# ucuapps/OpenGlue

Hardware: NVIDIA H100
Metric: image-pairs/sec at N=M=2048, d=256, 9 GNN layers, 100 Sinkhorn iters (higher is better)
Workload: dtype fp16x3 (fp16 hi/lo operands with power-of-two tensor scales, 3 products, fp32 accumulate)

## Files before the change

openglue_b200/csrc/attention_sm90.cuh:

```cuda
#pragma once
#include "tc_common.cuh"
#include <math_constants.h>

namespace og {

struct TcAttnArgs {
  const float* q; int64_t ldq, strideq;
  float* out; int64_t ldo, strideo;
  int batch, nq, nk, num_heads, d;
  float scale;
  const int* klen;
};

struct F16AttnScales {
  const float* q_amax;
  const float* k_scale;
  const float* v_scale;
  float* out_amax;
  int swap_halves;
};

namespace tca {
constexpr int BM = 128;
constexpr float LOG2E = 1.4426950408889634f;
constexpr float P_SHIFT = 14.f;
template <int DH, bool F16> struct Cfg {
  static constexpr int ESZ = F16 ? 2 : 4;
  static constexpr int BOX = 128 / ESZ;
  static constexpr int BNK = F16 ? 128 : 64;
  static constexpr int THREADS = F16 ? 384 : 256;
  static constexpr int K_TILE = BNK * DH * ESZ;
  static constexpr int V_TILE = DH * BNK * ESZ;
  static constexpr int STAGE = 2 * K_TILE + 2 * V_TILE;
  static constexpr int STAGES = 3;
  static constexpr int SMEM_BYTES = 1024 + STAGES * STAGE + 128;
  static_assert(SMEM_BYTES <= OG_SMEM_OPTIN_MAX, "dynamic shared memory of one block");
};
}

template <int ROWS, int STEP_BYTES>
__device__ __forceinline__ uint64_t tile_desc(uint32_t tile, int kk) {
  const int byte = kk * STEP_BYTES;
  return tc::make_wgdesc_sw128(tile + (byte >> 7) * ROWS * 128 + (byte & 127));
}

template <int DH, bool F16>
__device__ __forceinline__ void attention_issue(uint8_t* st, uint64_t* full, const CUtensorMap* mkh, const CUtensorMap* mkl,
                                                const CUtensorMap* mvh, const CUtensorMap* mvl, const TcAttnArgs& a, int h, int b,
                                                int i) {
  using C = tca::Cfg<DH, F16>;
  tc::mbar_arrive_expect_tx(full, C::STAGE);
#pragma unroll
  for (int j = 0; j < DH / C::BOX; ++j) {
    tc::tma_load_2d(st + j * C::BNK * 128, mkh, full, h * DH + j * C::BOX, b * a.nk + i * C::BNK);
    tc::tma_load_2d(st + C::K_TILE + j * C::BNK * 128, mkl, full, h * DH + j * C::BOX, b * a.nk + i * C::BNK);
  }
#pragma unroll
  for (int j = 0; j < C::BNK / C::BOX; ++j) {
    tc::tma_load_2d(st + 2 * C::K_TILE + j * DH * 128, mvh, full, i * C::BNK + j * C::BOX, b * a.d + h * DH);
    tc::tma_load_2d(st + 2 * C::K_TILE + C::V_TILE + j * DH * 128, mvl, full, i * C::BNK + j * C::BOX, b * a.d + h * DH);
  }
}

template <int NJ, bool F16>
__device__ __forceinline__ void attention_softmax(float (&p)[4 * NJ], int k0, int t, int nk, float c1, float (&m_run)[2],
                                                  float (&mc_run)[2], float (&l_run)[2], float (&corr)[2]) {
  using namespace tca;
  if (k0 + 8 * NJ > nk) {
    const int kbase = k0 + 2 * t;
#pragma unroll
    for (int j = 0; j < NJ; ++j)
#pragma unroll
      for (int e = 0; e < 4; ++e) if (kbase + 8 * j + (e & 1) >= nk) p[4 * j + e] = -CUDART_INF_F;
  }
#pragma unroll
  for (int hh = 0; hh < 2; ++hh) {
    float mx = -CUDART_INF_F;
#pragma unroll
    for (int j = 0; j < NJ; ++j) mx = fmaxf(mx, fmaxf(p[4 * j + 2 * hh], p[4 * j + 2 * hh + 1]));
    mx = fmaxf(mx, __shfl_xor_sync(0xffffffffu, mx, 1));
    mx = fmaxf(mx, __shfl_xor_sync(0xffffffffu, mx, 2));
    const float m_new = fmaxf(m_run[hh], mx);
    const float mc = F16 ? fmaf(m_new, c1, -P_SHIFT) : m_new * c1;
    corr[hh] = ex2_approx(mc_run[hh] - mc);
    float r = 0.f;
#pragma unroll
    for (int j = 0; j < NJ; ++j) {
#pragma unroll
      for (int e = 0; e < 2; ++e) {
        float& x = p[4 * j + 2 * hh + e];
        x = ex2_approx(fmaf(x, c1, -mc));
        r += x;
      }
    }
    l_run[hh] = fmaf(l_run[hh], corr[hh], r);
    m_run[hh] = m_new; mc_run[hh] = mc;
  }
}

template <int DH>
__device__ __forceinline__ float attention_store(const float (&acc)[DH / 2], const float (&l_run)[2], float inv_sv, int qr, int t,
                                                 const TcAttnArgs& a, int h, int b) {
  float omax = 0.f;
#pragma unroll
  for (int hh = 0; hh < 2; ++hh) {
    float l = l_run[hh];
    l += __shfl_xor_sync(0xffffffffu, l, 1);
    l += __shfl_xor_sync(0xffffffffu, l, 2);
    const float inv = inv_sv / l;
    const int row = qr + 8 * hh;
    if (row >= a.nq) continue;
    float* orow = a.out + (int64_t)b * a.strideo + (int64_t)row * a.ldo + h * DH;
#pragma unroll
    for (int j = 0; j < DH / 8; ++j) {
      const float2 v = make_float2(acc[4 * j + 2 * hh] * inv, acc[4 * j + 2 * hh + 1] * inv);
      *reinterpret_cast<float2*>(orow + 8 * j + 2 * t) = v;
      omax = fmaxf(omax, fmaxf(fabsf(v.x), fabsf(v.y)));
    }
  }
  return omax;
}

template <int DH>
__device__ __forceinline__ void attention_f16_ws(const CUtensorMap* mkh, const CUtensorMap* mkl, const CUtensorMap* mvh,
                                                 const CUtensorMap* mvl, const TcAttnArgs& a, const F16AttnScales& sc,
                                                 uint8_t* smem) {
  using namespace tca;
  using namespace tc;
  using C = Cfg<DH, true>;
  constexpr int S = C::STAGES, BNK = C::BNK;
  constexpr int QK = DH / 16, PK = BNK / 16, NJ = BNK / 8;
  constexpr int TURN = 1;
  static_assert(DH * 2 == 128, "one 128-byte row per K row");
  uint64_t* full = reinterpret_cast<uint64_t*>(smem + S * C::STAGE);
  uint64_t* empty = full + S;
  volatile uint32_t* timeout_flag = reinterpret_cast<uint32_t*>(empty + S);

  const int q0 = blockIdx.x * BM, h = blockIdx.y, b = blockIdx.z;
  const int nk = padded_length(a.klen, b, a.nk);
  const int nblk = cdiv(nk, BNK);
  const int wg = threadIdx.x >> 7;
  if (threadIdx.x == 0) {
    for (int i = 0; i < S; ++i) { mbar_init(&full[i], 1); mbar_init(&empty[i], 2); }
    *timeout_flag = 0;
    fence_barrier_init();
    prefetch_tensormap(mkh); prefetch_tensormap(mkl);
    prefetch_tensormap(mvh); prefetch_tensormap(mvl);
  }
  __syncthreads();
  grid_dependency_wait();

  if (wg == 0) {
    setmaxnreg_dec<24>();
    if (threadIdx.x == 0) {
      for (int i = 0; i < nblk; ++i) {
        const int s = i % S;
        if (i >= S) mbar_wait(&empty[s], (i / S - 1) & 1);
        attention_issue<DH, true>(smem + s * C::STAGE, &full[s], mkh, mkl, mvh, mvl, a, h, b, i);
      }
      mbar_wait(&empty[(nblk - 1) % S], ((nblk - 1) / S) & 1);
      if (*timeout_flag) asm volatile("trap;");
    }
    return;
  }
  setmaxnreg_inc<240>();
  const int c = wg - 1, tid = threadIdx.x & 127, warp = tid >> 5, lane = tid & 31, g = lane >> 2, t = lane & 3;
  const float s_q = f16_scale_for(__ldcg(sc.q_amax));
  const float c1 = a.scale * LOG2E / (s_q * __ldcg(sc.k_scale));
  const float inv_sv = 1.f / __ldcg(sc.v_scale);

  const float* qb = a.q + (int64_t)b * a.strideq + h * DH;
  uint32_t qh[QK][4], ql[QK][4];
#pragma unroll
  for (int kk = 0; kk < QK; ++kk)
#pragma unroll
    for (int e = 0; e < 4; ++e) {
      const int grow = q0 + c * 64 + warp * 16 + g + (e & 1) * 8, col = kk * 16 + 2 * t + (e >> 1) * 8;
      const float2 v = grow < a.nq ? *reinterpret_cast<const float2*>(qb + (int64_t)grow * a.ldq + col) : make_float2(0.f, 0.f);
      split_f16x2(v.x * s_q, v.y * s_q, qh[kk][e], ql[kk][e]);
    }

  float acc[DH / 2], o[DH / 2], p[4 * NJ];
#pragma unroll
  for (int k = 0; k < DH / 2; ++k) acc[k] = 0.f;
  float m_run[2] = {-CUDART_INF_F, -CUDART_INF_F}, mc_run[2] = {-CUDART_INF_F, -CUDART_INF_F}, l_run[2] = {0.f, 0.f};
  float corr[2];
  uint32_t phi[PK][4], plo[PK][4];
  uint32_t timed_out = 0;

  auto issue_qk = [&](int s) {
    const uint32_t khi = smem_u32(smem + s * C::STAGE), klo = khi + C::K_TILE;
#pragma unroll
    for (int kk = 0; kk < QK; ++kk) {
      const uint64_t bh = tile_desc<BNK, 32>(khi, kk), bl = tile_desc<BNK, 32>(klo, kk);
      wgmma_f16_m64n128(p, ql[kk], bh, kk ? 1 : 0);
      wgmma_f16_m64n128(p, qh[kk], bl, 1);
      wgmma_f16_m64n128(p, qh[kk], bh, 1);
    }
  };
  auto issue_pv = [&](int s) {
    const uint32_t vhi = smem_u32(smem + s * C::STAGE) + 2 * C::K_TILE, vlo = vhi + C::V_TILE;
#pragma unroll
    for (int kk = 0; kk < PK; ++kk) {
      const uint64_t dhi = tile_desc<DH, 32>(vhi, kk), dlo = tile_desc<DH, 32>(vlo, kk);
      wgmma_f16_m64n64(o, plo[kk], dhi, kk ? 1 : 0);
      wgmma_f16_m64n64(o, phi[kk], dlo, 1);
      wgmma_f16_m64n64(o, phi[kk], dhi, 1);
    }
  };
  auto split_p = [&]() {
#pragma unroll
    for (int kk = 0; kk < PK; ++kk)
#pragma unroll
      for (int e = 0; e < 4; ++e) {
        const int base = 4 * (2 * kk + (e >> 1)) + 2 * (e & 1);
        split_f16x2(p[base], p[base + 1], phi[kk][e], plo[kk][e]);
        if (sc.swap_halves) { phi[kk][e] = __byte_perm(phi[kk][e], 0, 0x1032); plo[kk][e] = __byte_perm(plo[kk][e], 0, 0x1032); }
      }
  };
  auto release_and_fold = [&](int s) {
    if (tid == 0) mbar_arrive(&empty[s]);
#pragma unroll
    for (int k = 0; k < DH / 2; ++k) acc[k] = fmaf(acc[k], corr[(k >> 1) & 1], o[k]);
  };

  if (c == 1) named_bar_arrive(TURN + 0, 256);
  mbar_wait_flag(&full[0], 0, timed_out);
  named_bar_sync(TURN + c, 256);
  fence_operands(p);
  wgmma_fence();
  issue_qk(0);
  wgmma_commit();
  named_bar_arrive(TURN + (c ^ 1), 256);
  wgmma_wait<0>();
  fence_operands(p);
  attention_softmax<NJ, true>(p, 0, t, nk, c1, m_run, mc_run, l_run, corr);
  split_p();

#pragma unroll 1
  for (int i = 1; i < nblk; ++i) {
    const int s = i % S, sp = (i - 1) % S;
    mbar_wait_flag(&full[s], (i / S) & 1, timed_out);
    named_bar_sync(TURN + c, 256);
    fence_operands(p);
    fence_operands(o);
    wgmma_fence();
    issue_qk(s);
    issue_pv(sp);
    wgmma_commit();
    named_bar_arrive(TURN + (c ^ 1), 256);
    wgmma_wait<0>();
    fence_operands(p);
    fence_operands(o);
    release_and_fold(sp);
    attention_softmax<NJ, true>(p, i * BNK, t, nk, c1, m_run, mc_run, l_run, corr);
    split_p();
  }

  if (timed_out) *timeout_flag = 1;
  named_bar_sync(TURN + c, 256);
  fence_operands(o);
  wgmma_fence();
  issue_pv((nblk - 1) % S);
  wgmma_commit();
  if (c == 0) named_bar_arrive(TURN + 1, 256);
  wgmma_wait<0>();
  fence_operands(o);
  release_and_fold((nblk - 1) % S);

  float omax = attention_store<DH>(acc, l_run, inv_sv, q0 + c * 64 + warp * 16 + g, t, a, h, b);
  if (sc.out_amax) {
    omax = warp_max(omax);
    if (lane == 0 && omax > 0.f) atomic_amax(sc.out_amax, omax);
  }
}

template <int DH>
__device__ __forceinline__ void attention_tf32(const CUtensorMap* mkh, const CUtensorMap* mkl, const CUtensorMap* mvh,
                                               const CUtensorMap* mvl, const TcAttnArgs& a, uint8_t* smem) {
  using namespace tca;
  using namespace tc;
  using C = Cfg<DH, false>;
  constexpr int S = C::STAGES, BNK = C::BNK;
  constexpr int QK = DH / 8;
  uint64_t* full = reinterpret_cast<uint64_t*>(smem + S * C::STAGE);
  uint64_t* empty = full + S;

  const int q0 = blockIdx.x * BM, h = blockIdx.y, b = blockIdx.z;
  const int nk = padded_length(a.klen, b, a.nk);
  const int nblk = cdiv(nk, BNK);
  const int wg = threadIdx.x >> 7, warp = (threadIdx.x >> 5) & 3, lane = threadIdx.x & 31, g = lane >> 2, t = lane & 3;
  if (threadIdx.x == 0) {
    for (int i = 0; i < S; ++i) { mbar_init(&full[i], 1); mbar_init(&empty[i], 8); }
    fence_barrier_init();
    prefetch_tensormap(mkh); prefetch_tensormap(mkl);
    prefetch_tensormap(mvh); prefetch_tensormap(mvl);
  }
  __syncthreads();
  grid_dependency_wait();

  if (threadIdx.x == 0)
    for (int i = 0; i < S && i < nblk; ++i) attention_issue<DH, false>(smem + i * C::STAGE, &full[i], mkh, mkl, mvh, mvl, a, h, b, i);

  const int qr = q0 + wg * 64 + warp * 16 + g;
  const float c1 = a.scale * LOG2E;
  const float* qb = a.q + (int64_t)b * a.strideq + h * DH;
  uint32_t qhi[QK][4], qlo[QK][4];
#pragma unroll
  for (int kk = 0; kk < QK; ++kk) {
#pragma unroll
    for (int e = 0; e < 4; ++e) {
      const int row = qr + (e & 1) * 8;
      const int col = kk * 8 + t + (e >> 1) * 4;
      split_tf32(row < a.nq ? qb[(int64_t)row * a.ldq + col] : 0.f, qhi[kk][e], qlo[kk][e]);
    }
  }

  float acc[DH / 2];
#pragma unroll
  for (int k = 0; k < DH / 2; ++k) acc[k] = 0.f;
  float m_run[2] = {-CUDART_INF_F, -CUDART_INF_F}, mc_run[2] = {-CUDART_INF_F, -CUDART_INF_F}, l_run[2] = {0.f, 0.f};

#pragma unroll 1
  for (int i = 0; i < nblk; ++i) {
    if (threadIdx.x == 0 && i >= 1 && i - 1 + S < nblk) {
      const int sr = (i - 1) % S;
      mbar_wait(&empty[sr], ((i - 1) / S) & 1);
      attention_issue<DH, false>(smem + sr * C::STAGE, &full[sr], mkh, mkl, mvh, mvl, a, h, b, i - 1 + S);
    }
    const int s = i % S;
    mbar_wait(&full[s], (i / S) & 1);
    const uint32_t st = smem_u32(smem + s * C::STAGE);
    const uint32_t khi = st, klo = st + C::K_TILE, vhi = st + 2 * C::K_TILE, vlo = vhi + C::V_TILE;

    float p[32];
    fence_operands(p);
    wgmma_fence();
#pragma unroll
    for (int kk = 0; kk < QK; ++kk) {
      const uint64_t dhi = tile_desc<BNK, 32>(khi, kk), dlo = tile_desc<BNK, 32>(klo, kk);
      wgmma_tf32_m64n64(p, qlo[kk], dhi, kk ? 1 : 0);
      wgmma_tf32_m64n64(p, qhi[kk], dlo, 1);
      wgmma_tf32_m64n64(p, qhi[kk], dhi, 1);
    }
    wgmma_commit();
    wgmma_wait<0>();
    fence_operands(p);

    float corr[2];
    attention_softmax<8, false>(p, i * BNK, t, nk, c1, m_run, mc_run, l_run, corr);

    float o[DH / 2];
    const int src0 = (lane & ~3) | (t >> 1), src1 = src0 + 2;
    const bool odd = t & 1;
#pragma unroll
    for (int half = 0; half < 2; ++half) {
      uint32_t phi[4][4], plo[4][4];
#pragma unroll
      for (int jj = 0; jj < 4; ++jj) {
        const int j = half * 4 + jj;
#pragma unroll
        for (int e = 0; e < 4; ++e) {
          const int reg = 4 * j + 2 * (e & 1), src = (e >> 1) ? src1 : src0;
          const float x0 = __shfl_sync(0xffffffffu, p[reg], src), x1 = __shfl_sync(0xffffffffu, p[reg + 1], src);
          split_tf32(odd ? x1 : x0, phi[jj][e], plo[jj][e]);
        }
      }
      fence_operands(o);
      wgmma_fence();
#pragma unroll
      for (int jj = 0; jj < 4; ++jj) {
        const int kk = half * 4 + jj;
        const uint64_t dhi = tile_desc<DH, 32>(vhi, kk), dlo = tile_desc<DH, 32>(vlo, kk);
        if constexpr (DH == 64) {
          wgmma_tf32_m64n64(o, plo[jj], dhi, kk ? 1 : 0);
          wgmma_tf32_m64n64(o, phi[jj], dlo, 1);
          wgmma_tf32_m64n64(o, phi[jj], dhi, 1);
        } else {
          wgmma_tf32_m64n32(o, plo[jj], dhi, kk ? 1 : 0);
          wgmma_tf32_m64n32(o, phi[jj], dlo, 1);
          wgmma_tf32_m64n32(o, phi[jj], dhi, 1);
        }
      }
      wgmma_commit();
      wgmma_wait<0>();
      fence_operands(o);
    }
    __syncwarp();
    if (lane == 0) mbar_arrive(&empty[s]);
#pragma unroll
    for (int k = 0; k < DH / 2; ++k) acc[k] = fmaf(acc[k], corr[(k >> 1) & 1], o[k]);
  }
  attention_store<DH>(acc, l_run, 1.f, qr, t, a, h, b);
}

template <int DH, bool F16>
__global__ void __launch_bounds__(tca::Cfg<DH, F16>::THREADS, 1) attention_sm90_kernel(const __grid_constant__ CUtensorMap map_khi,
                                                                                       const __grid_constant__ CUtensorMap map_klo,
                                                                                       const __grid_constant__ CUtensorMap map_vhi,
                                                                                       const __grid_constant__ CUtensorMap map_vlo,
                                                                                       TcAttnArgs a, F16AttnScales sc) {
  static_assert(DH == 64 || (DH == 32 && !F16), "head_dim 64 (both forms) or 32 (tf32)");
  tc::launch_dependents();
  extern __shared__ uint8_t og_att_smem_raw[];
  uint8_t* smem = tc::align_smem_1024(og_att_smem_raw);
  if constexpr (F16) attention_f16_ws<DH>(&map_khi, &map_klo, &map_vhi, &map_vlo, a, sc, smem);
  else attention_tf32<DH>(&map_khi, &map_klo, &map_vhi, &map_vlo, a, smem);
}

template <int DH, bool F16, class T>
inline int attention_sm90_launch(const TcAttnArgs& a, const F16AttnScales& sc, const T* khi, const T* klo, int64_t ldk,
                                 const T* vthi, const T* vtlo, int64_t ldvt, cudaStream_t stream) {
  using namespace tca;
  using C = Cfg<DH, F16>;
  CUtensorMap mkh, mkl, mvh, mvl;
  int rc;
  if ((rc = tc::make_tmap_2d(&mkh, khi, (uint64_t)a.batch * a.nk, (uint64_t)a.d, (uint64_t)ldk, C::BNK)) != OG_OK) return rc;
  if ((rc = tc::make_tmap_2d(&mkl, klo, (uint64_t)a.batch * a.nk, (uint64_t)a.d, (uint64_t)ldk, C::BNK)) != OG_OK) return rc;
  if ((rc = tc::make_tmap_2d(&mvh, vthi, (uint64_t)a.batch * a.d, (uint64_t)a.nk, (uint64_t)ldvt, DH)) != OG_OK) return rc;
  if ((rc = tc::make_tmap_2d(&mvl, vtlo, (uint64_t)a.batch * a.d, (uint64_t)a.nk, (uint64_t)ldvt, DH)) != OG_OK) return rc;
  if ((rc = smem_opt_in<attention_sm90_kernel<DH, F16>>(C::SMEM_BYTES, true)) != OG_OK) return rc;
  return launch("attention_sm90_kernel", attention_sm90_kernel<DH, F16>, LaunchAttr::pdl, dim3(cdiv(a.nq, BM), a.num_heads, a.batch),
                dim3(C::THREADS), C::SMEM_BYTES, stream, mkh, mkl, mvh, mvl, a, sc);
}

inline bool attention_tc_eligible(int head_dim, int64_t ldq, int64_t ldk, int64_t ldvt, int64_t ldo) {
  return (head_dim == 32 || head_dim == 64) && ldq % 2 == 0 && ldk % 4 == 0 && ldvt % 4 == 0 && ldo % 2 == 0;
}
inline int attention_tc_launch(const TcAttnArgs& a, const float* khi, const float* klo, int64_t ldk, const float* vthi,
                               const float* vtlo, int64_t ldvt, int head_dim, cudaStream_t stream) {
  const F16AttnScales none{nullptr, nullptr, nullptr, nullptr, 0};
  if (head_dim == 64) return attention_sm90_launch<64, false>(a, none, khi, klo, ldk, vthi, vtlo, ldvt, stream);
  if (head_dim == 32) return attention_sm90_launch<32, false>(a, none, khi, klo, ldk, vthi, vtlo, ldvt, stream);
  return fail(OG_EUNSUPPORTED, "attention_tc: head_dim %d not in {32, 64}", head_dim);
}

inline bool attention_f16_eligible(int head_dim, int64_t ldq, int64_t ldk, int64_t ldvt, int64_t ldo) {
  return head_dim == 64 && ldq % 2 == 0 && ldk % 8 == 0 && ldvt % 8 == 0 && ldo % 2 == 0;
}
inline int attention_f16_launch(const TcAttnArgs& a, const F16AttnScales& sc, const __half* khi, const __half* klo, int64_t ldk,
                                const __half* vthi, const __half* vtlo, int64_t ldvt, int head_dim, cudaStream_t stream) {
  if (head_dim != 64) return fail(OG_EUNSUPPORTED, "attention_f16: head_dim %d != 64", head_dim);
  if (!sc.q_amax || !sc.k_scale || !sc.v_scale) return fail(OG_EINVAL, "attention_f16: operand scales missing");
  return attention_sm90_launch<64, true>(a, sc, khi, klo, ldk, vthi, vtlo, ldvt, stream);
}

}
```

Baseline: 506.4.

## Make fp16 warp-specialized attention kernel persistent over query tiles

```diff
diff --git a/openglue_b200/csrc/attention_sm90.cuh b/openglue_b200/csrc/attention_sm90.cuh
--- a/openglue_b200/csrc/attention_sm90.cuh
+++ b/openglue_b200/csrc/attention_sm90.cuh
@@ -121,6 +121,19 @@
   return omax;
 }
 
+struct AttnTile {
+  int q0, h, b, nk;
+};
+__device__ __forceinline__ AttnTile attention_tile(const TcAttnArgs& a, int tile) {
+  const unsigned nqt = cdiv(a.nq, tca::BM), rest = (unsigned)tile / nqt, b = rest / (unsigned)a.num_heads;
+  AttnTile t;
+  t.q0 = (int)(tile - rest * nqt) * tca::BM;
+  t.h = (int)(rest - b * a.num_heads);
+  t.b = (int)b;
+  t.nk = padded_length(a.klen, t.b, a.nk);
+  return t;
+}
+
 template <int DH>
 __device__ __forceinline__ void attention_f16_ws(const CUtensorMap* mkh, const CUtensorMap* mkl, const CUtensorMap* mvh,
                                                  const CUtensorMap* mvl, const TcAttnArgs& a, const F16AttnScales& sc,
@@ -136,9 +149,7 @@
   uint64_t* empty = full + S;
   volatile uint32_t* timeout_flag = reinterpret_cast<uint32_t*>(empty + S);
 
-  const int q0 = blockIdx.x * BM, h = blockIdx.y, b = blockIdx.z;
-  const int nk = padded_length(a.klen, b, a.nk);
-  const int nblk = cdiv(nk, BNK);
+  const int tiles = cdiv(a.nq, BM) * a.num_heads * a.batch;
   const int wg = threadIdx.x >> 7;
   if (threadIdx.x == 0) {
     for (int i = 0; i < S; ++i) { mbar_init(&full[i], 1); mbar_init(&empty[i], 2); }
@@ -153,12 +164,16 @@
   if (wg == 0) {
     setmaxnreg_dec<24>();
     if (threadIdx.x == 0) {
-      for (int i = 0; i < nblk; ++i) {
-        const int s = i % S;
-        if (i >= S) mbar_wait(&empty[s], (i / S - 1) & 1);
-        attention_issue<DH, true>(smem + s * C::STAGE, &full[s], mkh, mkl, mvh, mvl, a, h, b, i);
-      }
-      mbar_wait(&empty[(nblk - 1) % S], ((nblk - 1) / S) & 1);
+      int it = 0;
+      for (int tile = blockIdx.x; tile < tiles; tile += gridDim.x) {
+        const AttnTile tl = attention_tile(a, tile);
+        for (int i = 0; i < cdiv(tl.nk, BNK); ++i, ++it) {
+          const int s = it % S;
+          if (it >= S) mbar_wait(&empty[s], (it / S - 1) & 1);
+          attention_issue<DH, true>(smem + s * C::STAGE, &full[s], mkh, mkl, mvh, mvl, a, tl.h, tl.b, i);
+        }
+      }
+      mbar_wait(&empty[(it - 1) % S], ((it - 1) / S) & 1);
       if (*timeout_flag) asm volatile("trap;");
     }
     return;
@@ -168,22 +183,37 @@
   const float s_q = f16_scale_for(__ldcg(sc.q_amax));
   const float c1 = a.scale * LOG2E / (s_q * __ldcg(sc.k_scale));
   const float inv_sv = 1.f / __ldcg(sc.v_scale);
-
-  const float* qb = a.q + (int64_t)b * a.strideq + h * DH;
+  const int row0 = c * 64 + warp * 16 + g;
+
   uint32_t qh[QK][4], ql[QK][4];
-#pragma unroll
-  for (int kk = 0; kk < QK; ++kk)
-#pragma unroll
-    for (int e = 0; e < 4; ++e) {
-      const int grow = q0 + c * 64 + warp * 16 + g + (e & 1) * 8, col = kk * 16 + 2 * t + (e >> 1) * 8;
-      const float2 v = grow < a.nq ? *reinterpret_cast<const float2*>(qb + (int64_t)grow * a.ldq + col) : make_float2(0.f, 0.f);
-      split_f16x2(v.x * s_q, v.y * s_q, qh[kk][e], ql[kk][e]);
-    }
+  auto load_q = [&](int tile) {
+    const AttnTile tl = attention_tile(a, tile);
+    const float* qb = a.q + (int64_t)tl.b * a.strideq + tl.h * DH;
+#pragma unroll
+    for (int kk = 0; kk < QK; ++kk)
+#pragma unroll
+      for (int e = 0; e < 4; ++e) {
+        const int grow = tl.q0 + row0 + (e & 1) * 8, col = kk * 16 + 2 * t + (e >> 1) * 8;
+        const float2 v = grow < a.nq ? *reinterpret_cast<const float2*>(qb + (int64_t)grow * a.ldq + col) : make_float2(0.f, 0.f);
+        qh[kk][e] = __float_as_uint(v.x);
+        ql[kk][e] = __float_as_uint(v.y);
+      }
+  };
+  auto split_q = [&]() {
+#pragma unroll
+    for (int kk = 0; kk < QK; ++kk)
+#pragma unroll
+      for (int e = 0; e < 4; ++e) split_f16x2(__uint_as_float(qh[kk][e]) * s_q, __uint_as_float(ql[kk][e]) * s_q, qh[kk][e], ql[kk][e]);
+  };
 
   float acc[DH / 2], o[DH / 2], p[4 * NJ];
-#pragma unroll
-  for (int k = 0; k < DH / 2; ++k) acc[k] = 0.f;
-  float m_run[2] = {-CUDART_INF_F, -CUDART_INF_F}, mc_run[2] = {-CUDART_INF_F, -CUDART_INF_F}, l_run[2] = {0.f, 0.f};
+  float m_run[2], mc_run[2], l_run[2];
+  auto reset = [&]() {
+#pragma unroll
+    for (int k = 0; k < DH / 2; ++k) acc[k] = 0.f;
+#pragma unroll
+    for (int hh = 0; hh < 2; ++hh) { m_run[hh] = -CUDART_INF_F; mc_run[hh] = -CUDART_INF_F; l_run[hh] = 0.f; }
+  };
   float corr[2];
   uint32_t phi[PK][4], plo[PK][4];
   uint32_t timed_out = 0;
@@ -223,56 +253,69 @@
 #pragma unroll
     for (int k = 0; k < DH / 2; ++k) acc[k] = fmaf(acc[k], corr[(k >> 1) & 1], o[k]);
   };
+  auto store = [&](int tile) {
+    const AttnTile tl = attention_tile(a, tile);
+    float omax = attention_store<DH>(acc, l_run, inv_sv, tl.q0 + row0, t, a, tl.h, tl.b);
+    if (sc.out_amax) {
+      omax = warp_max(omax);
+      if (lane == 0 && omax > 0.f) atomic_amax(sc.out_amax, omax);
+    }
+  };
+
+  int tile = blockIdx.x;
+  int nk = attention_tile(a, tile).nk;
+  load_q(tile);
+  split_q();
+  reset();
 
   if (c == 1) named_bar_arrive(TURN + 0, 256);
-  mbar_wait_flag(&full[0], 0, timed_out);
-  named_bar_sync(TURN + c, 256);
-  fence_operands(p);
-  wgmma_fence();
-  issue_qk(0);
-  wgmma_commit();
-  named_bar_arrive(TURN + (c ^ 1), 256);
-  wgmma_wait<0>();
-  fence_operands(p);
-  attention_softmax<NJ, true>(p, 0, t, nk, c1, m_run, mc_run, l_run, corr);
-  split_p();
-
+  int it = 0;
 #pragma unroll 1
-  for (int i = 1; i < nblk; ++i) {
-    const int s = i % S, sp = (i - 1) % S;
-    mbar_wait_flag(&full[s], (i / S) & 1, timed_out);
+  for (int i = 0;; ++it, ++i) {
+    const int s = it % S;
+    mbar_wait_flag(&full[s], (it / S) & 1, timed_out);
     named_bar_sync(TURN + c, 256);
     fence_operands(p);
     fence_operands(o);
     wgmma_fence();
     issue_qk(s);
-    issue_pv(sp);
+    if (it > 0) issue_pv((it - 1) % S);
     wgmma_commit();
     named_bar_arrive(TURN + (c ^ 1), 256);
     wgmma_wait<0>();
     fence_operands(p);
     fence_operands(o);
-    release_and_fold(sp);
+    if (it > 0) {
+      release_and_fold((it - 1) % S);
+      if (i == 0) {
+        store(tile - gridDim.x);
+        reset();
+      }
+    }
+    const bool last = i == cdiv(nk, BNK) - 1, more = tile + (int)gridDim.x < tiles;
     attention_softmax<NJ, true>(p, i * BNK, t, nk, c1, m_run, mc_run, l_run, corr);
     split_p();
+    if (last) {
+      if (!more) break;
+      tile += gridDim.x;
+      nk = attention_tile(a, tile).nk;
+      i = -1;
+      load_q(tile);
+      split_q();
+    }
   }
 
   if (timed_out) *timeout_flag = 1;
   named_bar_sync(TURN + c, 256);
   fence_operands(o);
   wgmma_fence();
-  issue_pv((nblk - 1) % S);
+  issue_pv(it % S);
   wgmma_commit();
   if (c == 0) named_bar_arrive(TURN + 1, 256);
   wgmma_wait<0>();
   fence_operands(o);
-  release_and_fold((nblk - 1) % S);
-
-  float omax = attention_store<DH>(acc, l_run, inv_sv, q0 + c * 64 + warp * 16 + g, t, a, h, b);
-  if (sc.out_amax) {
-    omax = warp_max(omax);
-    if (lane == 0 && omax > 0.f) atomic_amax(sc.out_amax, omax);
-  }
+  release_and_fold(it % S);
+  store(tile);
 }
 
 template <int DH>
@@ -420,8 +463,13 @@
   if ((rc = tc::make_tmap_2d(&mvh, vthi, (uint64_t)a.batch * a.d, (uint64_t)a.nk, (uint64_t)ldvt, DH)) != OG_OK) return rc;
   if ((rc = tc::make_tmap_2d(&mvl, vtlo, (uint64_t)a.batch * a.d, (uint64_t)a.nk, (uint64_t)ldvt, DH)) != OG_OK) return rc;
   if ((rc = smem_opt_in<attention_sm90_kernel<DH, F16>>(C::SMEM_BYTES, true)) != OG_OK) return rc;
-  return launch("attention_sm90_kernel", attention_sm90_kernel<DH, F16>, LaunchAttr::pdl, dim3(cdiv(a.nq, BM), a.num_heads, a.batch),
-                dim3(C::THREADS), C::SMEM_BYTES, stream, mkh, mkl, mvh, mvl, a, sc);
+  dim3 grid(cdiv(a.nq, BM), a.num_heads, a.batch);
+  if (F16) {
+    const int tiles = cdiv(a.nq, BM) * a.num_heads * a.batch;
+    grid = dim3(std::min(tiles, device_info().ok ? device_info().sm_count : 132));
+  }
+  return launch("attention_sm90_kernel", attention_sm90_kernel<DH, F16>, LaunchAttr::pdl, grid, dim3(C::THREADS), C::SMEM_BYTES, stream,
+                mkh, mkl, mvh, mvl, a, sc);
 }
 
 inline bool attention_tc_eligible(int head_dim, int64_t ldq, int64_t ldk, int64_t ldvt, int64_t ldo) {
```

Result: no change. 505.7 (median of 6 runs) (-0.1%).
